# tenstack/batch-scheduler

Hardware: AMD Instinct MI355X
Metric: pod x node fit evals/sec (higher is better)
Workload: dtype int64; 1 GPU; cfg3/tail: 10000 pods / 2000 groups / 5000 nodes, 5 int64 lanes (cpu, mem, eph, pods, gpu), seed 20260921; stages=prefilter+filter+tally+ready, parallelism=single GPU

## Files before the change

### batch-scheduler_amd/csrc/bs_fast.hpp

```cpp
#pragma once

#include "bs_kernels.hpp"
#include "bs_filter_t.hpp"

#ifdef BS_NT_TABLES
#define BS_TBL_STORE(p, v) __builtin_nontemporal_store((v), (p))
#else
#define BS_TBL_STORE(p, v) (*(p) = (v))
#endif
namespace bs {

template <bool INL = false>
__device__ __forceinline__ void arm_tally(const GroupsDev& gr, const BatchDev& b, const BatchParams& prm, uint32_t i, uint32_t nthreads);

__device__ __forceinline__ const uint8_t* range_glocal(const BatchDev& b) { return reinterpret_cast<const uint8_t*>(b.pod_ranges); }
__device__ __forceinline__ const uint32_t* range_start(const BatchDev& b, uint32_t G) { return b.pod_ranges + (G + 3u) / 4u; }
__device__ __forceinline__ const uint32_t* range_lfirst(const BatchDev& b, uint32_t G, uint32_t pod_blocks) { return range_start(b, G) + pod_blocks + 1u; }
__device__ __forceinline__ bool range_local_on(const BatchDev& b, const BatchParams& prm) {
  return b.pod_ranges && prm.do_tally && prm.do_ready && !prm.filter_deny;
}

#if BS_EMIT_MAIN
__global__ void k_pods_prep(unsigned long long* tables, uint32_t ntab, uint32_t* gstat, uint32_t ngstat, uint32_t* kcount, uint32_t* gcount, uint32_t G) {
  const uint32_t t = blockIdx.x * blockDim.x + threadIdx.x, nt = gridDim.x * blockDim.x;
// ... 476 lines not shown
    if (have && lp.have_mr) res_add(ms, lp.mr, sh, gate);
    uint32_t ff = (have && lp.have_mr) ? 1u : 0u;
#pragma unroll
    for (uint32_t q = 0; q < BS_MAX_SCALARS; ++q)
      if (q < sh.S() && (ms.present & (1u << q)) && ms.v[4 + q] != 0) ff |= 2u;
    const unsigned long long holds = __ballot(l[0] >= ms.v[0] && l[1] >= ms.v[1] && l[2] >= ms.v[2] && l[3] >= ms.v[3]);
    if (stores) {
      b.nodew[nodew_pair(stride, s, w)] = ok;
      b.nodew[nodew_pair(stride, s, w) + 1] = ~holds;
    }
    if (blk == 0 && threadIdx.x == 0) {
#pragma unroll
      for (int j = 0; j < 4; ++j) b.nodew[nodew_ref_lane(stride, s, j)] = (uint64_t)ms.v[j];
      b.nodew[nodew_ref_flags(stride, s)] = ff;
    }
  }
}

template <int TS>
__global__ __launch_bounds__(kTblChunk) void k_fast_query_tables(PodsDev pods, GroupsDev gr, NodesDev nd, BatchDev b, BatchDev bt, BatchParams prm,
                                                                 const TableDesc* forced, uint32_t nchunks, uint32_t query_blocks) {
  BS_STAMP(1, 0);
  if (blockIdx.x < query_blocks) fast_query_thread<TS>(pods, gr, b, prm, blockIdx.x * kTblChunk + threadIdx.x, query_blocks * kTblChunk);
  else if (blockIdx.x < query_blocks + nchunks) tables_local_fast<TS>(nd, bt, prm, forced, blockIdx.x - query_blocks);
  else node_words_block<TS>(gr, nd, b, prm, blockIdx.x - query_blocks - nchunks);
  BS_STAMP(1, 7);
}

template <int NL>
__device__ __forceinline__ unsigned long long rows_cover(unsigned long long m, const int64_t (&a)[BS_MAX_LANES], const int64_t (&r)[BS_MAX_LANES]) {
  asm volatile("s_mov_b64 exec, %[m]\n\tv_cmpx_ge_i64 vcc, %[a0], %[r0]\n\tv_cmpx_ge_i64 vcc, %[a1], %[r1]\n\tv_cmpx_ge_i64 vcc, %[a2], %[r2]\n\t"
               "v_cmpx_ge_i64 vcc, %[a3], %[r3]\n\ts_mov_b64 %[m], exec\n\ts_mov_b64 exec, -1"
               : [m] "+s"(m)
               : [a0] "v"(a[0]), [r0] "v"(r[0]), [a1] "v"(a[1]), [r1] "v"(r[1]), [a2] "v"(a[2]), [r2] "v"(r[2]), [a3] "v"(a[3]), [r3] "v"(r[3])
               : "vcc");
#pragma unroll
  for (int j = 4; j < NL; ++j)
    asm volatile("s_mov_b64 exec, %[m]\n\tv_cmpx_ge_i64 vcc, %[a], %[r]\n\ts_mov_b64 %[m], exec\n\ts_mov_b64 exec, -1" : [m] "+s"(m) : [a] "v"(a[j]), [r] "v"(r[j]) : "vcc");
  return m;
}
#ifndef BS_SCAN_BALLOT
#define BS_SCAN_BALLOT 1
#endif
constexpr uint32_t kSpinBound = 1u << 18;
__device__ __forceinline__ void test_chaos_delay() {
#ifdef BS_TEST_CHAOS
  uint32_t h = (blockIdx.x + 1u) * 2654435761u ^ (uint32_t)wall_clock64() * 40503u;
  h ^= h >> 15; h *= 2246822519u; h ^= h >> 13;
  for (uint32_t s = 0; s < (h & 15u); ++s) __builtin_amdgcn_s_sleep(127);
#endif
}
constexpr uint32_t kStepSlotsMax = 256;
__device__ __forceinline__ bool step_wait(const uint32_t* word, uint32_t base, uint32_t need, int32_t* h_err) {
  uint32_t spins = 0;
  while ((uint32_t)(ld_agent(word) - base) < need) {
    __builtin_amdgcn_s_sleep(1);
    if (++spins > kSpinBound) { if (h_err) __hip_atomic_store(h_err, 1, __ATOMIC_RELAXED, __HIP_MEMORY_SCOPE_SYSTEM); return false; }
  }
  return true;
}
constexpr uint32_t kScanRecChunks = 64;
constexpr uint32_t kFeasRecGroups = 32;
#ifndef BS_GATHER_DIRECT
#define BS_GATHER_DIRECT 8
#endif
constexpr uint32_t kGatherDirectBlocks = BS_GATHER_DIRECT;
constexpr uint32_t kRecStride = 32;
constexpr uint32_t kTkSlots = 32, kTkTab = 48, kTkP1 = 64, kTkDone = 64 + 16 * 16, kTkWays = 16, kTkWords = 64 + 2 * 16 * 16;
__device__ __forceinline__ void spread_add(uint32_t* words, uint32_t who) {
  (void)__hip_atomic_fetch_add(&words[16u * (who % kTkWays)], 1u, __ATOMIC_RELAXED, __HIP_MEMORY_SCOPE_AGENT);
}
__device__ __forceinline__ bool spread_wait(const uint32_t* words, uint32_t base, uint32_t need, int32_t* h_err) {
  uint32_t spins = 0;
  for (;;) {
    uint32_t v = lane_id() < (int)kTkWays ? ld_agent(&words[16u * (uint32_t)lane_id()]) : 0u;
#pragma unroll
    for (int o = 1; o < (int)kTkWays; o <<= 1) v += (uint32_t)__shfl_xor((int)v, o);
    v = (uint32_t)__builtin_amdgcn_readfirstlane((int)v);
    if ((uint32_t)(v - base) >= need) return true;
    __builtin_amdgcn_s_sleep(4);
    if (++spins > kSpinBound) { if (h_err && lane_id() == 0) __hip_atomic_store(h_err, 1, __ATOMIC_RELAXED, __HIP_MEMORY_SCOPE_SYSTEM); return false; }
  }
}
template <int TS, bool REGS = false>
__device__ __forceinline__ void table_scan_block(const NodesDev& nd, const BatchDev& b, const BatchParams& prm, const TableDesc* forced, uint32_t chunk, uint32_t nchunks,
                                                 uint32_t share, uint32_t nshares, uint32_t pod_blocks, uint32_t tk_pods0, uint32_t tk_tab0, const GroupsDev& gr,
                                                 const int64_t* ckeys, const uint32_t* cpres, uint32_t kcap, bool direct = false, uint32_t forced_cls = 0) {
  __shared__ unsigned long long s_wtot[BS_MAX_LANES][4];
  __shared__ uint32_t s_kp[BS_MAX_SCALARS];
  __shared__ unsigned long long s_off[BS_MAX_LANES];
  __shared__ uint32_t s_kpg[BS_MAX_SCALARS];
  __shared__ int64_t s_req[kStepSlotsMax][BS_MAX_LANES];
  __shared__ uint32_t s_qf[kStepSlotsMax];
  __shared__ uint32_t s_first[kStepSlotsMax];
  BS_STAMP(2, 0);
  const Shape<TS> sh(prm.S);
  const uint32_t L = sh.L(), S = sh.S(), LP = prm.LP;
  const uint32_t k = chunk * kTblChunk + threadIdx.x;
  const bool in_range = REGS ? k < nd.n : k < nd.m;
  const uint32_t n = REGS ? (in_range ? k : 0u) : (in_range ? nd.kmap[k] : 0u);
  const TableDesc d = REGS ? TableDesc{forced_cls, 0.7f} : *forced;
  const uint32_t fw = nd.fit[(size_t)d.cls * nd.fit_words + (n >> 5)];
  const uint8_t fl = nd.flags[n];
  const bool valid = in_range && (!REGS || !(fl & BS_NODE_SKIP_MASK));
  const uint32_t ap = nd.apres[n], rp = nd.rpres[n];
  int64_t al[BS_MAX_LANES], rq[BS_MAX_LANES];
#pragma unroll
  for (uint32_t j = 0; j < BS_MAX_LANES; ++j) {
    if (j < L) {
      al[j] = nd.alloc[(size_t)j * nd.stride + n];
      rq[j] = nd.req[(size_t)j * nd.stride + n];
    }
  }
  const uint32_t K = prm.k_host ? prm.k_host : *b.kclass;
  const uint32_t per = (K + nshares - 1u) / nshares, s_lo = share * per, s_hi = min(K, s_lo + per);
  Res raw;
  int32_t leader0 = -1;
  uint8_t panic0 = 0;
  LeaderPre lp0{};
  if constexpr (REGS) {
    const uint32_t cc = s_lo + threadIdx.x < s_hi ? s_lo + threadIdx.x : 0u;
#pragma unroll
    for (uint32_t j = 0; j < BS_MAX_LANES; ++j)
      if (j < L) raw.v[j] = ckeys[(size_t)j * kcap + cc];
    raw.present = cpres[cc];
    leader0 = b.leader_epoch[0];
    panic0 = b.panic_epoch[0];
    if (gr.g) leader_pre_load(gr, leader0, sh, lp0);
  }
  const bool fit = valid && ((fw >> (n & 31u)) & 1u) && !(fl & BS_NODE_TAINT_ERR);
  const uint32_t pres = fit ? (ap & rp) : 0u;
  if (threadIdx.x < BS_MAX_SCALARS) s_kp[threadIdx.x] = BS_INF;
  for (uint32_t t = threadIdx.x; t < kStepSlotsMax; t += kTblChunk) s_first[t] = BS_INF;
  unsigned long long incl[BS_MAX_LANES];
  const int w = wave_id();
#pragma unroll
  for (uint32_t j = 0; j < BS_MAX_LANES; ++j) {
    incl[j] = 0;
    if (j < L) {
      const bool live = fit && (j < 4 || (pres & (1u << (j - 4)))) && !(j == BS_LANE_EPH && !prm.eph_gate);
      const unsigned long long left = live ? (unsigned long long)wsub(scale_f32(al[j], d.pct), rq[j]) : 0ull;
      incl[j] = wave_incl_scan_add_u64(left);
      if (lane_id() == 63) s_wtot[j][w] = incl[j];
    }
  }
  __syncthreads();
#pragma unroll
  for (uint32_t s2 = 0; s2 < BS_MAX_SCALARS; ++s2) {
    if (s2 < S) {
      const unsigned long long mk = __ballot(valid && (pres & (1u << s2)));
      if (mk && lane_id() == 0) atomicMin(&s_kp[s2], chunk * kTblChunk + (uint32_t)(threadIdx.x & ~63u) + (uint32_t)(__ffsll((long long)mk) - 1));
    }
  }
#pragma unroll
  for (uint32_t j = 0; j < BS_MAX_LANES; ++j) {
    if (j < L) {
      unsigned long long off = 0, tot = 0;
#pragma unroll
      for (int i = 0; i < 4; ++i) {
        const unsigned long long x = s_wtot[j][i];
        if (i < w) off += x;
        tot += x;
      }
      incl[j] += off;
      if (threadIdx.x == 0 && share == 0) {
        if constexpr (REGS) {
          const unsigned long long tag = (unsigned long long)prm.seq_inv << 32;
          st_pub<true>(&b.chunk_rec[(size_t)chunk * kRecStride + 2u * j], tag | (uint32_t)tot);
          st_pub<true>(&b.chunk_rec[(size_t)chunk * kRecStride + 2u * j + 1u], tag | (uint32_t)(tot >> 32));
        } else {
          st_pub<true>(&b.chunk_tot[(size_t)chunk * 16 + j], tot);
        }
      }
    }
  }
  __syncthreads();
  __shared__ uint32_t s_ok;
  if constexpr (REGS) {
    if (share == 0 && threadIdx.x < S) st_pub<true>(&b.chunk_rec[(size_t)chunk * kRecStride + 16u + threadIdx.x], ((unsigned long long)prm.seq_inv << 32) | s_kp[threadIdx.x]);
    BS_STAMP(2, 1);
  } else {
    if (share == 0 && threadIdx.x < 16) st_pub<true>(&b.chunk_kp[(size_t)chunk * 16 + threadIdx.x], threadIdx.x < BS_MAX_SCALARS ? s_kp[threadIdx.x] : BS_INF);
    asm volatile("s_waitcnt vmcnt(0)" ::: "memory");
    __syncthreads();
    BS_STAMP(2, 1);
    if (threadIdx.x == 0 && share == 0) (void)__hip_atomic_fetch_add(&b.ticket[kTkTab], 1u, __ATOMIC_RELAXED, __HIP_MEMORY_SCOPE_AGENT);
  }
  if constexpr (REGS) {
    const uint32_t t = s_lo + threadIdx.x;
    if (t < s_hi) {
      uint32_t qf = 0x80000000u;
      Res q;
      res_zero(q, sh);
      if (leader0 >= 0 && !panic0) {
        Res cur;
        res_zero(cur, sh);
        res_add(cur, raw, sh, prm.eph_gate);
        qf = class_scan_query(cur, lp0, sh, prm.eph_gate, q);
      }
      s_qf[threadIdx.x] = qf;
#pragma unroll
      for (uint32_t j = 0; j < BS_MAX_LANES; ++j)
        if (j < L) s_req[threadIdx.x][j] = q.v[j];
    }
  }
  if constexpr (!REGS) {
    if (threadIdx.x == 0) s_ok = (step_wait(&b.ticket[kTkTab], tk_tab0, nchunks, b.h_err) && step_wait(&b.ticket[kTkSlots], tk_pods0, pod_blocks, b.h_err)) ? 1u : 0u;
    __syncthreads();
    BS_STAMP(2, 2);
    if (!s_ok) return;
  }
  {
    const uint32_t ch = (uint32_t)lane_id();
    unsigned long long cv[BS_MAX_LANES];
    uint32_t ckp[BS_MAX_SCALARS];
    if constexpr (REGS) {
      if (w == 0) {
        const uint32_t tagw = prm.seq_inv;
        const unsigned long long* rec = b.chunk_rec + (size_t)(ch < nchunks ? ch : 0u) * kRecStride;
        bool ok = false;
        for (uint32_t spins = 0;; ++spins) {
          unsigned long long lo[BS_MAX_LANES], hi[BS_MAX_LANES], kw[BS_MAX_SCALARS];
#pragma unroll
          for (uint32_t j = 0; j < BS_MAX_LANES; ++j)
            if (j < L) { lo[j] = ld_agent64(&rec[2u * j]); hi[j] = ld_agent64(&rec[2u * j + 1u]); }
#pragma unroll
          for (uint32_t s2 = 0; s2 < BS_MAX_SCALARS; ++s2)
            if (s2 < S) kw[s2] = ld_agent64(&rec[16u + s2]);
          bool mine_ok = true;
#pragma unroll
          for (uint32_t j = 0; j < BS_MAX_LANES; ++j) {
            cv[j] = 0ull;
            if (j < L) {
              mine_ok = mine_ok && (uint32_t)(lo[j] >> 32) == tagw && (uint32_t)(hi[j] >> 32) == tagw;
              cv[j] = (hi[j] << 32) | (uint32_t)lo[j];
            }
          }
#pragma unroll
          for (uint32_t s2 = 0; s2 < BS_MAX_SCALARS; ++s2) {
            ckp[s2] = BS_INF;
            if (s2 < S) { mine_ok = mine_ok && (uint32_t)(kw[s2] >> 32) == tagw; ckp[s2] = (uint32_t)kw[s2]; }
          }
          if (__ballot(!(mine_ok || ch >= nchunks)) == 0ull) { ok = true; break; }
          if (spins > kSpinBound) { if (b.h_err && ch == 0) __hip_atomic_store(b.h_err, 1, __ATOMIC_RELAXED, __HIP_MEMORY_SCOPE_SYSTEM); break; }
          __builtin_amdgcn_s_sleep(2);
        }
        if (ch >= nchunks) {
#pragma unroll
          for (uint32_t j = 0; j < BS_MAX_LANES; ++j) cv[j] = 0ull;
#pragma unroll
          for (uint32_t s2 = 0; s2 < BS_MAX_SCALARS; ++s2) ckp[s2] = BS_INF;
        }
        if (ch == 0) s_ok = ok ? 1u : 0u;
      }
      BS_STAMP(2, 2);
    } else if (w == 0) {
#pragma unroll
      for (uint32_t j = 0; j < BS_MAX_LANES; ++j) cv[j] = (j < L && ch < nchunks) ? ld_agent64(&b.chunk_tot[(size_t)ch * 16 + j]) : 0ull;
#pragma unroll
      for (uint32_t s2 = 0; s2 < BS_MAX_SCALARS; ++s2) ckp[s2] = (s2 < S && ch < nchunks) ? ld_agent(&b.chunk_kp[(size_t)ch * 16 + s2]) : BS_INF;
    }
    const uint32_t t = s_lo + threadIdx.x;
    uint32_t stp = 0, qf = 0x80000000u;
    int32_t tab = -1;
    unsigned long long rv[BS_MAX_LANES];
    if (!REGS && t < s_hi) {
      stp = ld_agent(&b.qstamp_s[t]);
      tab = (int32_t)ld_agent(reinterpret_cast<const uint32_t*>(&b.qtab_s[t]));
      qf = ld_agent(&b.qflags_s[t]);
#pragma unroll
      for (uint32_t j = 0; j < BS_MAX_LANES; ++j) rv[j] = j < L ? ld_agent64(&b.qreq_s[(size_t)t * LP + j]) : 0ull;
    }
    if (w == 0) {
#pragma unroll
      for (uint32_t j = 0; j < BS_MAX_LANES; ++j) {
        if (j < L) {
          const unsigned long long incl_c = wave_incl_scan_add_u64(cv[j]);
          const unsigned long long mine = bcast64(incl_c - cv[j], (int)(chunk & 63u));
          if (ch == 0) s_off[j] = mine;
        }
      }
#pragma unroll
      for (uint32_t s2 = 0; s2 < BS_MAX_SCALARS; ++s2) {
        if (s2 < S) {
          const uint32_t mn = wave_min_u32(ckp[s2]);
          if (ch == 0) s_kpg[s2] = mn;
        }
      }
    }
    if (!REGS && t < s_hi) {
      if (stp != prm.stamp || tab != 0) qf = 0x80000000u;
      s_qf[threadIdx.x] = qf;
#pragma unroll
      for (uint32_t j = 0; j < BS_MAX_LANES; ++j)
        if (j < L) s_req[threadIdx.x][j] = (int64_t)rv[j];
    }
  }
  __syncthreads();
  if constexpr (REGS) {
    if (!s_ok) return;
  }
  int64_t fin[BS_MAX_LANES];
  uint32_t keyrow = 0;
#pragma unroll
  for (uint32_t j = 0; j < BS_MAX_LANES; ++j) {
    fin[j] = 0;
    if (j < L) fin[j] = (int64_t)(incl[j] + s_off[j]);
  }
#pragma unroll
  for (uint32_t s2 = 0; s2 < BS_MAX_SCALARS; ++s2)
    if (s2 < S && k >= s_kpg[s2]) keyrow |= 1u << s2;
  BS_STAMP(2, 3);
  const uint32_t nmine = s_hi > s_lo ? s_hi - s_lo : 0u;
  const uint32_t smask = S ? ((1u << S) - 1u) : 0u;
  const uint32_t row0 = chunk * kTblChunk + ((uint32_t)w << 6);
  for (uint32_t t0 = 0; t0 < nmine; t0 += 4u) {
    uint32_t qf[4];
    int64_t r[4][BS_MAX_LANES];
#pragma unroll
    for (uint32_t u = 0; u < 4; ++u) {
      const uint32_t t = min(t0 + u, nmine - 1u);
      qf[u] = t0 + u < nmine ? s_qf[t] : 0x80000000u;
#pragma unroll
      for (uint32_t j = 0; j < BS_MAX_LANES; ++j) r[u][j] = j < L ? s_req[t][j] : 0;
    }
#pragma unroll
    for (uint32_t u = 0; u < 4; ++u) {
      const uint32_t nab = ~(qf[u] >> 16) & smask;
      unsigned long long m = (qf[u] & 0x80000000u) ? 0ull : __ballot(valid && (nab & ~keyrow) == 0u);
      static_assert(TS >= 0 && TS <= 4, "k_fast_step_a is instantiated for 0..4 scalar lanes (run_fast: step_a_possible)");
#if BS_SCAN_BALLOT
#pragma unroll
      for (uint32_t j = 0; j < 4u + (uint32_t)TS; ++j) m &= __ballot(fin[j] >= r[u][j]);
#else
      m = rows_cover<4 + TS>(m, fin, r[u]);
#endif
      if (m && lane_id() == 0) atomicMin(&s_first[t0 + u], row0 + (uint32_t)(__ffsll((long long)m) - 1));
    }
  }
  __syncthreads();
  BS_STAMP(2, 4);
  if constexpr (REGS) {
    if (direct) {
      for (uint32_t t = threadIdx.x; t < nmine; t += kTblChunk)
        st_pub<true>(&b.scan_rec[(size_t)chunk * kStepSlotsMax + s_lo + t], ((unsigned long long)prm.seq_inv << 32) | s_first[t]);
    } else {
      for (uint32_t t = threadIdx.x; t < nmine; t += kTblChunk)
        if (s_first[t] != BS_INF) atomicMin(&b.first_row64[s_lo + t], ((unsigned long long)prm.seq_inv << 32) | s_first[t]);
    }
    BS_STAMP(2, 7);
    return;
  }
  for (uint32_t t = threadIdx.x; t < nmine; t += kTblChunk) {
    if (s_first[t] == BS_INF) continue;
    atomicMin(&b.first_row[s_lo + t], s_first[t]);
  }
  BS_STAMP(2, 7);
}

__device__ __forceinline__ void step_filter_split(uint32_t K, uint32_t W, uint32_t target_waves, uint32_t& tiles, uint32_t& bpw, uint32_t& nchunk) {
  tiles = (2u * K + 63u) / 64u;
  uint32_t nsplit = max(1u, target_waves / max(tiles, 1u));
  nsplit = min(nsplit, max((W + 1u) / 2u, 1u));
  bpw = max(2u, (((W + nsplit - 1u) / nsplit + 1u) / 2u) * 2u);
  nchunk = (W + bpw - 1u) / bpw;
  if ((nchunk + 3u) / 4u > kFeasRecGroups) {
    bpw = ((W + 4u * kFeasRecGroups - 1u) / (4u * kFeasRecGroups) + 1u) / 2u * 2u;
    nchunk = (W + bpw - 1u) / bpw;
  }
}
template <int TS>
__device__ __forceinline__ void step_filter_block(const GroupsDev& gr, const NodesDev& nd, const BatchDev& b, const BatchParams& prm, const int64_t* ckeys,
                                                  const uint32_t* cpres, uint32_t kcap, uint32_t target_waves, uint32_t ustride, uint32_t bx, uint32_t nblocks,
                                                  bool direct, uint32_t tk_slots0, uint32_t slot_producers) {
  __shared__ uint32_t s_cnt[4][64];
  BS_STAMP_AT(4, 0, bx);
  const Shape<TS> sh(prm.S);
  const uint32_t gate = prm.eph_gate, K = prm.k_host ? prm.k_host : (uint32_t)__builtin_amdgcn_readfirstlane((int)*b.kclass), U = 2u * K;
  const uint32_t W = (nd.n + 63u) / 64u;
  if (!U || !W) return;
  uint32_t tiles, bpw, nchunk;
  step_filter_split(K, W, target_waves, tiles, bpw, nchunk);
  const uint32_t groups = (nchunk + 3u) / 4u;
  const int32_t leader0 = b.leader_epoch[0];
  LeaderPre lp0{}, lp1{};
  const bool two = prm.sop_leader0 >= 0 && prm.sop_leader0 != leader0;
  if (gr.g) {
    leader_pre_load(gr, leader0, sh, lp0);
    if (two) leader_pre_load(gr, prm.sop_leader0, sh, lp1); else lp1 = lp0;
  }
  bool waited = false;
  for (uint32_t bi = bx; bi < tiles * groups; bi += nblocks) {
    const uint32_t tile = bi % tiles, group = bi / tiles, chunk = group * 4u + (uint32_t)wave_id();
    const uint32_t src = tile * 64u + (uint32_t)lane_id();
    const bool second = src >= K;
    const uint32_t c = src < U ? (second ? src - K : src) : 0u;
    uint32_t cnt = 0;
    if (chunk < nchunk) {
      Res raw;
#pragma unroll
      for (uint32_t j = 0; j < BS_MAX_LANES; ++j)
        if (j < sh.L()) raw.v[j] = ckeys[(size_t)j * kcap + c];
      raw.present = cpres[c];
      Res cur;
      res_zero(cur, sh);
      res_add(cur, raw, sh, gate);
      LeaderPre lp = lp0;
      if (second) lp = lp1;
      const bool on = src < U && (second ? prm.sop_leader0 >= 0 : leader0 >= 0) && lp.have_mr;
      int64_t R[4], M[4];
      const uint32_t ff = filter_slot_values(cur, lp, sh, gate, R, M);
      filter_item<2, 4, true, true>(nd, b, U, ustride, tile, chunk * bpw, min(W, chunk * bpw + bpw), 0u,
                                    on ? (ff | ((uint32_t)BS_FL_EVALUATED << 8)) : ((uint32_t)BS_FL_NOT_RUN << 8), R, M, &cnt);
    }
    s_cnt[wave_id()][lane_id()] = cnt;
    BS_STAMP_AT(4, 1, bx);
    if (direct && b.h_rows) asm volatile("s_waitcnt vmcnt(0)" ::: "memory");
    __syncthreads();
    BS_STAMP_AT(4, 2, bx);
    if (wave_id() == 0 && src < U) {
      const uint32_t sum = s_cnt[0][lane_id()] + s_cnt[1][lane_id()] + s_cnt[2][lane_id()] + s_cnt[3][lane_id()];
      if (direct) {
        st_pub<true>(&b.feas_rec[(size_t)group * (2u * kStepSlotsMax) + src], ((unsigned long long)prm.seq_inv << 32) | sum);
      } else {
        if (!waited) { (void)step_wait(&b.ticket[kTkSlots], tk_slots0, slot_producers, b.h_err); waited = true; }
        if (sum) atomicAdd(&b.fu_feas[src], sum);
      }
    }
    __syncthreads();
  }
  BS_STAMP_AT(4, 7, bx);
}

template <int TS>
__device__ __forceinline__ void class_slots_block(const GroupsDev& gr, const BatchDev& b, const BatchParams& prm, const int64_t* ckeys, const uint32_t* cpres,
                                                  uint32_t kcap, uint32_t blk, bool zero_feas) {
  const Shape<TS> sh(prm.S);
#ifdef BS_TEST_OLD_ZERO
  zero_feas = true;
#endif
  const uint32_t gate = prm.eph_gate, K = prm.k_host ? prm.k_host : *b.kclass;
  const uint32_t c = blk * kTblChunk + threadIdx.x;
  Res raw;
  const uint32_t cc = c < K ? c : 0u;
#pragma unroll
  for (uint32_t j = 0; j < BS_MAX_LANES; ++j)
    if (j < sh.L()) raw.v[j] = ckeys[(size_t)j * kcap + cc];
  raw.present = cpres[cc];
  const int32_t leader0 = b.leader_epoch[0];
  const uint8_t panic0 = b.panic_epoch[0];
  LeaderPre lp0{}, lp1{};
  const bool two = prm.run_filter && prm.sop_leader0 >= 0 && prm.sop_leader0 != leader0;
  if (gr.g) {
    leader_pre_load(gr, leader0, sh, lp0);
    if (two) leader_pre_load(gr, prm.sop_leader0, sh, lp1); else lp1 = lp0;
  }
  if (c < K) {
    Res cur;
    res_zero(cur, sh);
    res_add(cur, raw, sh, gate);
    if (leader0 >= 0 && !panic0) {
      Res q;
      const uint32_t qfw = class_scan_query(cur, lp0, sh, gate, q);
      int64_t* dst = b.qreq_s + (size_t)c * prm.LP;
#pragma unroll
      for (uint32_t j = 0; j < BS_MAX_LANES; ++j)
        if (j < prm.LP) st_pub<true>(&dst[j], j < sh.L() ? q.v[j] : (int64_t)INT64_MIN);
      st_pub<true>(&b.qflags_s[c], qfw);
      st_pub<true>(&b.qtab_s[c], (int32_t)0);
      st_pub<true>(&b.first_row[c], BS_INF);
      st_pub<true>(&b.qstamp_s[c], prm.stamp);
    }
    if (prm.run_filter) {
      if (leader0 >= 0) filter_slot_from<TS, true>(b, prm, cur, lp0, sh, gate, c, zero_feas);
      if (prm.sop_leader0 >= 0) filter_slot_from<TS, true>(b, prm, cur, lp1, sh, gate, c + K, zero_feas);
    }
  }
  BS_STAMP(1, 4);
  asm volatile("s_waitcnt vmcnt(0)" ::: "memory");
  __syncthreads();
  BS_STAMP(1, 5);
  if (threadIdx.x == 0) (void)__hip_atomic_fetch_add(&b.ticket[kTkSlots], 1u, __ATOMIC_RELAXED, __HIP_MEMORY_SCOPE_AGENT);
}


template <bool INL>
__device__ __forceinline__ void arm_tally(const GroupsDev& gr, const BatchDev& b, const BatchParams& prm, uint32_t i, uint32_t nthreads) {
  if (i == 0) __hip_atomic_store(&b.ticket[1], 0u, __ATOMIC_RELAXED, __HIP_MEMORY_SCOPE_AGENT);
  for (uint32_t g = i; g < gr.g; g += nthreads) {
    if (INL && range_local_on(b, prm) && range_glocal(b)[g]) continue;
    st_pub<INL>(&b.admit[g], 0u);
    if (prm.do_ready) {
      st_pub<INL>(&b.admit64[g], 0ull);
      if (b.gcount[g] == 0u) {
        const uint8_t rd = gr.matched[g] >= (uint32_t)(gr.min_member[g] - gr.status_scheduled[g]) ? 1 : 0;
        b.ready[g] = rd;
        if (prm.host_tag) { st_home(&b.h_admit[g], 0u); st_home(&b.h_ready[g], rd); }
      }
    }
  }
}

template <bool WT = false>
__device__ __forceinline__ void final_tail(const BatchDev& b, const BatchParams& prm, uint32_t nblocks) {
  __shared__ uint32_t s_last;
  if (!prm.host_tag) return;
  if constexpr (WT && BS_HOME_WT) asm volatile("s_waitcnt vmcnt(0)" ::: "memory");
  else __builtin_amdgcn_fence(__ATOMIC_RELEASE, "");
// ... 292 lines not shown
      tally_tail<true>(gr, b, prm, grouped, grouped ? (uint32_t)gi0 : 0u, admit, nblocks);
  }
  BS_STAMP(3, 7);
}

template <int S>
__global__ __launch_bounds__(256) void k_fast_scan_filter(PodsDev pods, NodesDev nd, BatchDev bt, BatchParams prm, uint32_t m, uint32_t jcap,
                                                          uint32_t scan_blocks, uint32_t filter_waves, uint32_t ustride) {
  __shared__ int64_t s_rows[4][64][4 + S];
  if (blockIdx.x < scan_blocks)
    scan_loop<S, true, 1>(bt, prm, m, jcap, 0u, 0u, 1u, blockIdx.x, scan_blocks, s_rows[wave_id()]);
  else
    filter_loop<2>(pods, nd, bt, filter_waves, 1u, ustride, prm.collect_stats, blockIdx.x - scan_blocks, gridDim.x - scan_blocks, prm.stamp, 2u * prm.k_host);
}
template <int S>
__global__ __launch_bounds__(256) void k_fast_scan(BatchDev bt, BatchParams prm, uint32_t m, uint32_t jcap) {
  __shared__ int64_t s_rows[4][64][4 + S];
  scan_loop<S, true, 1>(bt, prm, m, jcap, 0u, 0u, 1u, blockIdx.x, gridDim.x, s_rows[wave_id()]);
}
template <int PU, bool DB>
__global__ __launch_bounds__(256) void k_fast_filter(PodsDev pods, NodesDev nd, BatchDev bt, BatchParams prm, uint32_t filter_waves, uint32_t ustride) {
  filter_loop<2, PU, DB>(pods, nd, bt, filter_waves, 1u, ustride, prm.collect_stats, blockIdx.x, gridDim.x, prm.stamp, 2u * prm.k_host);
}
#if BS_EMIT_FAST
__global__ __launch_bounds__(256) __attribute__((amdgpu_waves_per_eu(7))) void k_fast_filter_w7(PodsDev pods, NodesDev nd, BatchDev bt, BatchParams prm, uint32_t filter_waves,
                                                                                                uint32_t ustride) {
  filter_loop<2, 2, false>(pods, nd, bt, filter_waves, 1u, ustride, prm.collect_stats, blockIdx.x, gridDim.x, prm.stamp, 2u * prm.k_host);
}
#endif
#if BS_EMIT_FAST
__global__ __launch_bounds__(256) void k_fast_filter_t(NodesDev nd, BatchDev bt, BatchParams prm, uint32_t filter_waves, uint32_t ustride, uint32_t by_tile) {
  filter_loop_t<false>(nd, bt, filter_waves, ustride, prm.collect_stats, blockIdx.x, gridDim.x, prm.stamp, 2u * prm.k_host, by_tile);
}
#endif
template <int S>
__global__ __launch_bounds__(256) __attribute__((amdgpu_waves_per_eu(S <= 1 ? 4 : 1))) void k_fast_scan_filter_t(NodesDev nd, BatchDev bt, BatchParams prm, uint32_t m, uint32_t jcap, uint32_t scan_blocks,
                                                            uint32_t filter_waves, uint32_t ustride, uint32_t form) {
  __shared__ int64_t s_rows[4][64][4 + S];
  const uint32_t filter_first = form & 1u, by_tile = form & 2u;
  const uint32_t filter_blocks = gridDim.x - scan_blocks;
  const bool is_scan = filter_first ? blockIdx.x >= filter_blocks : blockIdx.x < scan_blocks;
  BS_STAMP(2, 0);
  if (is_scan)
    scan_loop<S, true, 1>(bt, prm, m, jcap, 0u, 0u, 1u, filter_first ? blockIdx.x - filter_blocks : blockIdx.x, scan_blocks, s_rows[wave_id()]);
  else
    filter_loop_t<true>(nd, bt, filter_waves, ustride, prm.collect_stats, filter_first ? blockIdx.x : blockIdx.x - scan_blocks, filter_blocks, prm.stamp, 2u * prm.k_host, by_tile);
  BS_STAMP(2, 7);
}
#if BS_EMIT_MAIN
__global__ __launch_bounds__(256) void k_fast_final(PodsDev pods, GroupsDev gr, NodesDev nd, BatchDev b, BatchParams prm, uint32_t query_blocks) {
  fast_final_block(pods, gr, nd, b, prm, query_blocks, blockIdx.x, gridDim.x, 0u);
}
#endif

template <int S>
__global__ __launch_bounds__(256) void k_fast_scan_filter_final(PodsDev pods, GroupsDev gr, NodesDev nd, BatchDev b, BatchDev bt, BatchParams prm, uint32_t m,
                                                                uint32_t jcap, uint32_t scan_blocks, uint32_t filter_blocks, uint32_t filter_waves,
                                                                uint32_t ustride, uint32_t query_blocks) {
  __shared__ int64_t s_rows[4][64][4 + S];
  const uint32_t producers = scan_blocks + filter_blocks;
  test_chaos_delay();
#ifdef BS_TEST_LATE_ROLE_B
  {
    const int role = blockIdx.x < scan_blocks ? 0 : blockIdx.x < producers ? 1 : 2;
    if (role == BS_TEST_LATE_ROLE_B) for (int spin = 0; spin < 20; ++spin) __builtin_amdgcn_s_sleep(127);
  }
#endif
  if (blockIdx.x < producers) {
    BS_STAMP(2, 0);
    if (blockIdx.x < scan_blocks)
      scan_loop<S, true, 2>(bt, prm, m, jcap, 0u, 0u, 1u, blockIdx.x, scan_blocks, s_rows[wave_id()]);
    else
      filter_loop<2>(pods, nd, bt, filter_waves, 1u, ustride, prm.collect_stats, blockIdx.x - scan_blocks, filter_blocks, prm.stamp, 2u * prm.k_host);
    asm volatile("s_waitcnt vmcnt(0)" ::: "memory");
    __syncthreads();
    if (threadIdx.x == 0) (void)__hip_atomic_fetch_add(&b.ticket[1], 1u, __ATOMIC_RELAXED, __HIP_MEMORY_SCOPE_AGENT);
    BS_STAMP(2, 7);
    return;
  }
  fast_final_block(pods, gr, nd, b, prm, query_blocks, blockIdx.x - producers, gridDim.x - producers, producers);
}

template <int TS, bool WHOLE>
__global__ __launch_bounds__(kTblChunk) void k_fast_step_a(PodsDev pods, GroupsDev gr, NodesDev nd, BatchDev b, BatchDev bt, BatchParams prm, const TableDesc* forced,
                                                           uint32_t nchunks, uint32_t query_blocks, uint32_t nshares, uint32_t filter_blocks, uint32_t filter_waves,
                                                           uint32_t ustride, uint32_t tk_pods0, uint32_t tk_tab0, uint32_t param_blocks, const int64_t* ckeys,
                                                           const uint32_t* cpres, uint32_t kcap, uint32_t tk_p1, uint32_t tk_done, uint32_t forced_cls) {
  BS_STAMP(1, 0);
  test_chaos_delay();
  const uint32_t tb = nchunks * nshares;
#ifdef BS_TEST_LATE_ROLE
  {
    const int role = blockIdx.x < query_blocks ? 0 : blockIdx.x < query_blocks + param_blocks ? 1 : blockIdx.x < query_blocks + param_blocks + tb ? 2 : 3;
    if (role == BS_TEST_LATE_ROLE) for (int spin = 0; spin < 20; ++spin) __builtin_amdgcn_s_sleep(127);
  }
#endif
  const uint32_t producers = param_blocks ? param_blocks : query_blocks;
  const bool direct = query_blocks <= kGatherDirectBlocks;
  if (blockIdx.x < query_blocks) {
    if constexpr (WHOLE) {
      const uint32_t p0 = b.pod_ranges ? range_start(b, gr.g)[blockIdx.x] : blockIdx.x * kTblChunk;
      const uint32_t p1 = b.pod_ranges ? range_start(b, gr.g)[blockIdx.x + 1u] : pods.p;
      fast_query_thread<TS, false, false, true>(pods, gr, b, prm, p0 + threadIdx.x, query_blocks * kTblChunk, p1, blockIdx.x * kTblChunk + threadIdx.x);
      asm volatile("s_waitcnt vmcnt(0)" ::: "memory");
      __syncthreads();
      if (threadIdx.x == 0) spread_add(&b.ticket[kTkP1], blockIdx.x);
      fast_final_block<true>(pods, gr, nd, b, prm, query_blocks, blockIdx.x, query_blocks, nchunks, tk_p1, filter_waves, tk_done, tb + filter_blocks, p0, p1);
    } else if (param_blocks) {
      fast_query_thread<TS, false, false>(pods, gr, b, prm, blockIdx.x * kTblChunk + threadIdx.x, query_blocks * kTblChunk);
    } else {
      fast_query_thread<TS, true>(pods, gr, b, prm, blockIdx.x * kTblChunk + threadIdx.x, query_blocks * kTblChunk);
      BS_STAMP(1, 4);
      asm volatile("s_waitcnt vmcnt(0)" ::: "memory");
      __syncthreads();
      BS_STAMP(1, 5);
      if (threadIdx.x == 0) (void)__hip_atomic_fetch_add(&b.ticket[kTkSlots], 1u, __ATOMIC_RELAXED, __HIP_MEMORY_SCOPE_AGENT);
    }
  } else if (blockIdx.x < query_blocks + param_blocks) {
    class_slots_block<TS>(gr, b, prm, ckeys, cpres, kcap, blockIdx.x - query_blocks, !(WHOLE && direct));
  } else if (blockIdx.x < query_blocks + param_blocks + tb) {
    const uint32_t x = blockIdx.x - query_blocks - param_blocks;
    table_scan_block<TS, WHOLE>(nd, bt, prm, forced, x / nshares, nchunks, x % nshares, nshares, producers, tk_pods0, tk_tab0, gr, ckeys, cpres, kcap, direct, forced_cls);
    if constexpr (WHOLE) {
      if (!direct) {
        asm volatile("s_waitcnt vmcnt(0)" ::: "memory");
        __syncthreads();
        if (threadIdx.x == 0) spread_add(&b.ticket[kTkDone], blockIdx.x);
      }
    }
  } else if constexpr (WHOLE) {
    step_filter_block<TS>(gr, nd, bt, prm, ckeys, cpres, kcap, filter_waves, ustride, blockIdx.x - query_blocks - param_blocks - tb, filter_blocks, direct, tk_pods0, producers);
    if (!direct) {
      asm volatile("s_waitcnt vmcnt(0)" ::: "memory");
      __syncthreads();
      if (threadIdx.x == 0) spread_add(&b.ticket[kTkDone], blockIdx.x);
    }
  } else {
    __shared__ uint32_t s_go;
    if (threadIdx.x == 0) {
      s_go = step_wait(&b.ticket[kTkSlots], tk_pods0, producers, b.h_err) ? 1u : 0u;
      __builtin_amdgcn_fence(__ATOMIC_ACQUIRE, "agent");
    }
    __syncthreads();
    if (!s_go) return;
    filter_loop<2>(pods, nd, bt, filter_waves, 1u, ustride, prm.collect_stats, blockIdx.x - query_blocks - param_blocks - tb, filter_blocks, prm.stamp, 2u * prm.k_host);
  }
  BS_STAMP(1, 7);
}


template <int TS>
__global__ __launch_bounds__(kTblChunk) void k_tables_local_nofix(NodesDev nd, BatchDev b, BatchParams prm, uint32_t nchunks, uint32_t cstride,
                                                                  uint32_t gstride) {
  const uint32_t slot = blockIdx.x;
  if (!b.needed[slot]) return;
  BatchDev bt = b;
  bt.tables = b.tables + (size_t)slot * prm.mcap * prm.LP;
  bt.kp = b.kp + (size_t)slot * 16;
  bt.chunk_tot = b.chunk_tot + (size_t)slot * cstride * 16;
  bt.chunk_kp = b.chunk_kp + (size_t)slot * cstride * 16;
  bt.gmax = b.gmax + (size_t)slot * gstride * prm.LP;
  const TableDesc d = table_desc(slot, prm.C, nullptr);
  tables_local_fast<TS>(nd, bt, prm, &d, blockIdx.y);
}

#if BS_EMIT_MAIN
__global__ __launch_bounds__(kLeaderBlock) void k_leader_scan(GroupsDev gr, BatchDev b) {
// ... 93 lines not shown
```

### batch-scheduler_amd/csrc/bs_kernels.hpp

```cpp
#pragma once

#include "bs_common.hpp"
#include "bs_nodew_layout.hpp"

namespace bs {

struct NodesDev {
  uint32_t n, stride;
  const int64_t* alloc;
  const int64_t* req;
  const uint32_t* apres;
  const uint32_t* rpres;
  const uint8_t* flags;
  const uint32_t* fit;
  uint32_t fit_words, n_classes;
  const uint32_t* kmap;
  uint32_t m;
  const int64_t* left4;
  const int64_t* lglob;
};

struct GroupsDev {
  uint32_t g;
  const uint32_t* min_member;
// ... 1486 lines not shown
__global__ void k_filter_params(PodsDev pods, GroupsDev gr, BatchDev b, BatchParams prm) {
  const uint32_t i = blockIdx.x * blockDim.x + threadIdx.x;
  if (i >= pods.p) return;
  filter_params_for<-1>(pods, gr, b, prm, i, b.pf_code[i], b.pf_leader[i], i, true, true);
}
#endif

template <int TS>
__global__ void k_fparams_early(PodsDev pods, GroupsDev gr, BatchDev b, BatchParams prm) {
  const uint32_t i = blockIdx.x * blockDim.x + threadIdx.x;
  if (i >= pods.p) return;
  const uint8_t pf = (b.stage[i] & ST_OWNED) ? b.tcode[i] : (uint8_t)BS_PF_NOT_OWNED;
  const bool after = i >= b.nepochs[1];
  const int32_t leader = after ? b.leader_epoch[0] : prm.sop_leader0;
  const uint32_t slot = prm.use_classes ? b.pclass[i] + (after ? 0u : *b.kclass) : i;
  filter_params_for<TS>(pods, gr, b, prm, i, pf, leader, slot, true, true);
}

#define BS_OPT_0(x) ""
#define BS_OPT_1(x) x
#define BS_OPT(flag, x) BS_OPT_##flag(x)
template <int MASK>
__device__ __forceinline__ void filter_pod2(uint32_t pp, const int64_t (&R)[4], unsigned long long ok0, unsigned long long ok1,
                                            const int64_t (&l0)[4], const int64_t (&l1)[4], uint32_t& vlo0, uint32_t& vhi0,
                                            uint32_t& vlo1, uint32_t& vhi1);
#define BS_DEF_FILTER_POD2(MASK, f0, f1, f2, f3)                                                                          \
  template <>                                                                                                             \
  __device__ __forceinline__ void filter_pod2<MASK>(uint32_t pp, const int64_t (&R)[4], unsigned long long ok0,          \
                                                    unsigned long long ok1, const int64_t (&l0)[4], const int64_t (&l1)[4], \
                                                    uint32_t& vlo0, uint32_t& vhi0, uint32_t& vlo1, uint32_t& vhi1) {       \
    asm volatile("s_mov_b32 m0, %[pp]\n\t"                                                                                \
                 "s_mov_b64 exec, %[ok0]\n\t"                                                                             \
                 BS_OPT(f0, "v_cmpx_le_i64 vcc, %[R0], %[a0]\n\t") BS_OPT(f1, "v_cmpx_le_i64 vcc, %[R1], %[a1]\n\t")       \
                 BS_OPT(f2, "v_cmpx_le_i64 vcc, %[R2], %[a2]\n\t") BS_OPT(f3, "v_cmpx_le_i64 vcc, %[R3], %[a3]\n\t")       \
                 "s_nop 3\n\t"                                                                                            \
                 "v_writelane_b32 %[vlo0], exec_lo, m0\n\t"                                                               \
                 "v_writelane_b32 %[vhi0], exec_hi, m0\n\t"                                                               \
                 "s_mov_b64 exec, %[ok1]\n\t"                                                                             \
                 BS_OPT(f0, "v_cmpx_le_i64 vcc, %[R0], %[b0]\n\t") BS_OPT(f1, "v_cmpx_le_i64 vcc, %[R1], %[b1]\n\t")       \
                 BS_OPT(f2, "v_cmpx_le_i64 vcc, %[R2], %[b2]\n\t") BS_OPT(f3, "v_cmpx_le_i64 vcc, %[R3], %[b3]\n\t")       \
                 "s_nop 3\n\t"                                                                                            \
                 "v_writelane_b32 %[vlo1], exec_lo, m0\n\t"                                                               \
                 "v_writelane_b32 %[vhi1], exec_hi, m0\n\t"                                                               \
                 "s_mov_b64 exec, -1"                                                                                     \
                 : [vlo0] "+v"(vlo0), [vhi0] "+v"(vhi0), [vlo1] "+v"(vlo1), [vhi1] "+v"(vhi1)                             \
                 : [pp] "s"(pp), [ok0] "s"(ok0), [ok1] "s"(ok1), [R0] "v"(R[0]), [R1] "v"(R[1]), [R2] "v"(R[2]),          \
                   [R3] "v"(R[3]), [a0] "v"(l0[0]), [a1] "v"(l0[1]), [a2] "v"(l0[2]), [a3] "v"(l0[3]), [b0] "v"(l1[0]),   \
                   [b1] "v"(l1[1]), [b2] "v"(l1[2]), [b3] "v"(l1[3])                                                      \
                 : "vcc");                                                                                                \
  }
BS_DEF_FILTER_POD2(1, 1, 0, 0, 0)
BS_DEF_FILTER_POD2(2, 0, 1, 0, 0)
BS_DEF_FILTER_POD2(3, 1, 1, 0, 0)
BS_DEF_FILTER_POD2(4, 0, 0, 1, 0)
BS_DEF_FILTER_POD2(5, 1, 0, 1, 0)
BS_DEF_FILTER_POD2(6, 0, 1, 1, 0)
BS_DEF_FILTER_POD2(7, 1, 1, 1, 0)
BS_DEF_FILTER_POD2(8, 0, 0, 0, 1)
BS_DEF_FILTER_POD2(9, 1, 0, 0, 1)
BS_DEF_FILTER_POD2(10, 0, 1, 0, 1)
BS_DEF_FILTER_POD2(11, 1, 1, 0, 1)
BS_DEF_FILTER_POD2(12, 0, 0, 1, 1)
BS_DEF_FILTER_POD2(13, 1, 0, 1, 1)
BS_DEF_FILTER_POD2(14, 0, 1, 1, 1)
BS_DEF_FILTER_POD2(15, 1, 1, 1, 1)

template <int MASK, int PU = 4>
__device__ __forceinline__ void filter_pod_loop(uint32_t np, const int64_t (*sR)[4], const unsigned long long (&okmask)[2],
                                                const int64_t (&l)[2][4], uint32_t (&vlo)[2], uint32_t (&vhi)[2]) {
  for (uint32_t pp = 0; pp < np; pp += PU) {
    int64_t R[PU][4];
#pragma unroll
    for (int u = 0; u < PU; ++u) {
      const uint32_t pu = min(pp + (uint32_t)u, np - 1);
#pragma unroll
      for (int j = 0; j < 4; ++j) R[u][j] = ((MASK >> j) & 1) ? sR[pu][j] : 0;
    }
#pragma unroll
    for (int u = 0; u < PU; ++u)
      filter_pod2<MASK>(min(pp + (uint32_t)u, np - 1), R[u], okmask[0], okmask[1], l[0], l[1], vlo[0], vhi[0], vlo[1], vhi[1]);
  }
}

template <int NB, int PU = 4, bool DB = true, bool REGS = false>
__device__ __forceinline__ void filter_item(const NodesDev& nd, const BatchDev& b, uint32_t U, uint32_t ustride, uint32_t ptile,
                                            uint32_t w0, uint32_t w1, uint32_t stamp = 0, uint32_t ff_in = 0, const int64_t* R_in = nullptr,
                                            const int64_t* M_in = nullptr, uint32_t* cnt_out = nullptr) {
  static_assert(NB == 2, "the inner statement handles two node blocks");
  typedef const __attribute__((address_space(4))) uint32_t* cflag_t;
  const int lane = lane_id();
  const uint32_t p0 = ptile * 64u;
  const uint32_t np = min(64u, U - p0);

  const bool mine = (uint32_t)lane < np;
  const uint32_t src = p0 + (uint32_t)lane;
  uint32_t myff = (uint32_t)BS_FL_NOT_RUN << 8;
  int64_t M[4] = {0, 0, 0, 0}, myR[4] = {0, 0, 0, 0};
  if constexpr (REGS) {
    if (mine) {
      myff = ff_in;
#pragma unroll
      for (int j = 0; j < 4; ++j) { myR[j] = R_in[j]; M[j] = M_in[j]; }
    }
  } else if (mine) {
    myff = b.uflags[src];
    const int64_t* rs = b.uparams + (size_t)src * 8;
#pragma unroll
    for (int j = 0; j < 4; ++j) { myR[j] = rs[j]; M[j] = rs[4 + j]; }
  }
  int64_t gl[8];
#pragma unroll
  for (int j = 0; j < 8; ++j) gl[j] = nd.lglob[j];
  int64_t l[NB][4], ln[NB][4];
  uint8_t nfl[NB], nfln[NB];
  auto load_blocks = [&](uint32_t w, int64_t (&dst)[NB][4], uint8_t (&fl)[NB]) {
#pragma unroll
    for (int nb = 0; nb < NB; ++nb) {
      const uint32_t n = (w + nb) * 64u + (uint32_t)lane;
      const bool nvalid = (w + nb) < w1 && n < nd.n;
      fl[nb] = 0xFF;
#pragma unroll
      for (int j = 0; j < 4; ++j) dst[nb][j] = INT64_MIN;
      if (nvalid) {
#pragma unroll
        for (int j = 0; j < 4; ++j) dst[nb][j] = nd.left4[(size_t)j * nd.stride + n];
        fl[nb] = nd.flags[n];
      }
    }
  };
  load_blocks(w0, l, nfl);
  if (!REGS && stamp) myff = (myff >> 16) == stamp ? (myff & 0xFFFFu) : ((uint32_t)BS_FL_NOT_RUN << 8);
  const uint32_t myfl = myff >> 8;
  const bool ev = myfl == BS_FL_EVALUATED;
  if (!ev) {
#pragma unroll
    for (int j = 0; j < 4; ++j) M[j] = 0;
  }
  __shared__ int64_t s_R[4][64][4];
  __builtin_amdgcn_wave_barrier();
  uint32_t lane_mask = 0;
  bool tile_allfail = false;
  {
#pragma unroll
    for (int j = 0; j < 4; ++j) s_R[wave_id()][lane][j] = myR[j];
    __builtin_amdgcn_wave_barrier();
    const bool c2pod = ev && !(myff & 1u);
    const unsigned long long c2mask = __ballot(c2pod);
#pragma unroll
    for (int j = 0; j < 4; ++j) {
      if (__ballot(c2pod && !(gl[j] >= myR[j]))) lane_mask |= 1u << j;
      if (c2mask && !__ballot(c2pod && gl[4 + j] >= myR[j])) tile_allfail = true;
    }
  }
  const unsigned long long evmask = __ballot(ev);
  if (!evmask) return;
  bool uniformM = true;
  int64_t M0[4] = {0, 0, 0, 0};
  uint32_t lb0 = 0;
  if (evmask) {
    const int first = __ffsll((long long)evmask) - 1;
    bool same = true;
#pragma unroll
    for (int j = 0; j < 4; ++j) {
      M0[j] = __shfl(M[j], first);
      same = same && (M[j] == M0[j]);
    }
    lb0 = (uint32_t)__shfl((int)(myff & 2u), first);
    same = same && ((myff & 2u) == lb0);
    uniformM = __ballot(ev && !same) == 0;
  }

  crow_t FP = as_const_rows(b.uparams);
  cflag_t FF = (cflag_t)(uintptr_t)b.uflags;
  uint32_t cnt = 0;
  for (uint32_t w = w0; w < w1; w += NB) {
    if constexpr (DB) {
      if (w + NB < w1) load_blocks(w + NB, ln, nfln);
    }
    unsigned long long okmask[NB], in_range[NB], nlf[NB];
    uint32_t vlo[NB], vhi[NB];
#pragma unroll
    for (int nb = 0; nb < NB; ++nb) {
      const bool nvalid = nfl[nb] != 0xFF;
      const bool node_ok = nvalid && !(nfl[nb] & (BS_NODE_NIL | BS_NODE_NO_NODE));
      in_range[nb] = __ballot(nvalid);
      okmask[nb] = __ballot(node_ok);
      unsigned long long lf = 0;
      if (!lb0) lf = __ballot(l[nb][0] >= M0[0]) & __ballot(l[nb][1] >= M0[1]) & __ballot(l[nb][2] >= M0[2]) & __ballot(l[nb][3] >= M0[3]);
      nlf[nb] = okmask[nb] & ~lf;
      vlo[nb] = 0;
      vhi[nb] = 0;
    }
    if (uniformM) {
      const int64_t (*sR)[4] = s_R[wave_id()];
      if (tile_allfail) {
      } else {
        switch (lane_mask) {
          case 0:
#pragma unroll
            for (int nb = 0; nb < NB; ++nb) { vlo[nb] = (uint32_t)okmask[nb]; vhi[nb] = (uint32_t)(okmask[nb] >> 32); }
            break;
          case 1: filter_pod_loop<1, PU>(np, sR, okmask, l, vlo, vhi); break;
          case 2: filter_pod_loop<2, PU>(np, sR, okmask, l, vlo, vhi); break;
          case 3: filter_pod_loop<3, PU>(np, sR, okmask, l, vlo, vhi); break;
          case 4: filter_pod_loop<4, PU>(np, sR, okmask, l, vlo, vhi); break;
          case 5: filter_pod_loop<5, PU>(np, sR, okmask, l, vlo, vhi); break;
          case 6: filter_pod_loop<6, PU>(np, sR, okmask, l, vlo, vhi); break;
          case 7: filter_pod_loop<7, PU>(np, sR, okmask, l, vlo, vhi); break;
          case 8: filter_pod_loop<8, PU>(np, sR, okmask, l, vlo, vhi); break;
          case 9: filter_pod_loop<9, PU>(np, sR, okmask, l, vlo, vhi); break;
          case 10: filter_pod_loop<10, PU>(np, sR, okmask, l, vlo, vhi); break;
          case 11: filter_pod_loop<11, PU>(np, sR, okmask, l, vlo, vhi); break;
          case 12: filter_pod_loop<12, PU>(np, sR, okmask, l, vlo, vhi); break;
// ... 281 lines not shown
```

Measured before the change: 3765 billion evals/s.

## Restructure step-A table scan with lane-distributed requests and prefetch filter inputs

In the REGS table-scan path, each lane now holds one pod request in registers, and the wave broadcasts it with readlane instead of rereading shared memory for every pod. Per-pod first-row results are collected into a lane via v_writelane and committed with one atomicMin per lane, replacing one atomic per pod. The filter loop also prefetches pod keys and node blocks for the next item before the leader preload and before waiting on the ticket, and it skips the spin-wait when an early ticket read already shows all producers are done. The kernel is additionally hinted to run at 3 waves per EU, which could cause register spills or lower occupancy.

```diff
diff --git a/batch-scheduler_amd/csrc/bs_fast.hpp b/batch-scheduler_amd/csrc/bs_fast.hpp
--- a/batch-scheduler_amd/csrc/bs_fast.hpp
+++ b/batch-scheduler_amd/csrc/bs_fast.hpp
@@ -582,6 +582,13 @@
     if (++spins > kSpinBound) { if (h_err && lane_id() == 0) __hip_atomic_store(h_err, 1, __ATOMIC_RELAXED, __HIP_MEMORY_SCOPE_SYSTEM); return false; }
   }
 }
+#pragma clang diagnostic push
+#pragma clang diagnostic ignored "-Winline-asm"
+__device__ __forceinline__ uint32_t writelane_sgpr(uint32_t value, int lane, uint32_t old) {
+  asm("s_mov_b32 m0, %2\n\tv_writelane_b32 %0, %1, m0" : "+v"(old) : "s"(value), "s"(lane) : "m0");
+  return old;
+}
+#pragma clang diagnostic pop
 template <int TS, bool REGS = false>
 __device__ __forceinline__ void table_scan_block(const NodesDev& nd, const BatchDev& b, const BatchParams& prm, const TableDesc* forced, uint32_t chunk, uint32_t nchunks,
                                                  uint32_t share, uint32_t nshares, uint32_t pod_blocks, uint32_t tk_pods0, uint32_t tk_tab0, const GroupsDev& gr,
@@ -704,6 +711,24 @@
         if (j < L) s_req[threadIdx.x][j] = q.v[j];
     }
   }
+  const uint32_t nmine = (uint32_t)__builtin_amdgcn_readfirstlane((int)(s_hi > s_lo ? s_hi - s_lo : 0u));
+  const uint32_t smask = S ? ((1u << S) - 1u) : 0u;
+  static_assert(TS >= 0 && TS <= 4, "k_fast_step_a is instantiated for 0..4 scalar lanes (run_fast: step_a_possible)");
+  constexpr uint32_t NL = 4u + (uint32_t)TS;
+  int64_t rr[NL];
+  uint32_t nabx = 0;
+  [[maybe_unused]] auto req_round = [&](uint32_t base) {
+    const uint32_t t = base + (uint32_t)lane_id();
+    const bool have = t < nmine;
+    const uint32_t qf = have ? s_qf[t] : 0x80000000u;
+#pragma unroll
+    for (uint32_t j = 0; j < NL; ++j) rr[j] = have ? s_req[t][j] : 0;
+    nabx = (qf & 0x80000000u) ? 0xC0000000u : ((~(qf >> 16) & smask) | 0x80000000u);
+  };
+  if constexpr (REGS) {
+    __syncthreads();
+    req_round(0u);
+  }
   if constexpr (!REGS) {
     if (threadIdx.x == 0) s_ok = (step_wait(&b.ticket[kTkTab], tk_tab0, nchunks, b.h_err) && step_wait(&b.ticket[kTkSlots], tk_pods0, pod_blocks, b.h_err)) ? 1u : 0u;
     __syncthreads();
@@ -811,9 +836,32 @@
   for (uint32_t s2 = 0; s2 < BS_MAX_SCALARS; ++s2)
     if (s2 < S && k >= s_kpg[s2]) keyrow |= 1u << s2;
   BS_STAMP(2, 3);
-  const uint32_t nmine = s_hi > s_lo ? s_hi - s_lo : 0u;
-  const uint32_t smask = S ? ((1u << S) - 1u) : 0u;
-  const uint32_t row0 = chunk * kTblChunk + ((uint32_t)w << 6);
+  const uint32_t row0 = (uint32_t)__builtin_amdgcn_readfirstlane((int)(chunk * kTblChunk + ((uint32_t)w << 6)));
+  if constexpr (REGS) {
+    constexpr uint32_t kU = TS <= 1 ? 8u : 4u;
+    const uint32_t rowbits = valid ? ((~keyrow & smask) | 0x40000000u) : ~0u;
+    for (uint32_t base = 0; base < nmine; base += 64u) {
+      if (base) req_round(base);
+      const uint32_t cnt = min(64u, nmine - base);
+      uint32_t first = BS_INF;
+      for (uint32_t s0 = 0; s0 < cnt; s0 += kU) {
+#pragma unroll
+        for (uint32_t u = 0; u < kU; ++u) {
+          const int sl = (int)(s0 + u);
+          unsigned long long m = __ballot(((uint32_t)__builtin_amdgcn_readlane((int)nabx, sl) & rowbits) == 0u);
+#pragma unroll
+          for (uint32_t j = 0; j < NL; ++j) {
+            const int64_t r = (int64_t)(((unsigned long long)(uint32_t)__builtin_amdgcn_readlane((int)((unsigned long long)rr[j] >> 32), sl) << 32) |
+                                        (uint32_t)__builtin_amdgcn_readlane((int)(uint32_t)rr[j], sl));
+            m &= __ballot(fin[j] >= r);
+          }
+          const uint32_t row = m ? row0 + (uint32_t)(__ffsll((long long)m) - 1) : BS_INF;
+          first = writelane_sgpr(row, sl, first);
+        }
+      }
+      if ((uint32_t)lane_id() < cnt && first != BS_INF) atomicMin(&s_first[base + (uint32_t)lane_id()], first);
+    }
+  } else {
   for (uint32_t t0 = 0; t0 < nmine; t0 += 4u) {
     uint32_t qf[4];
     int64_t r[4][BS_MAX_LANES];
@@ -837,6 +885,7 @@
 #endif
       if (m && lane_id() == 0) atomicMin(&s_first[t0 + u], row0 + (uint32_t)(__ffsll((long long)m) - 1));
     }
+  }
   }
   __syncthreads();
   BS_STAMP(2, 4);
@@ -883,25 +932,36 @@
   step_filter_split(K, W, target_waves, tiles, bpw, nchunk);
   const uint32_t groups = (nchunk + 3u) / 4u;
   const int32_t leader0 = b.leader_epoch[0];
+  Res raw;
+  FilterPre<2> pre;
+  auto item_load = [&](uint32_t bi) {
+    const uint32_t tile = bi % tiles, chunk = (bi / tiles) * 4u + (uint32_t)wave_id();
+    const uint32_t src = tile * 64u + (uint32_t)lane_id();
+    const uint32_t c = src < U ? (src >= K ? src - K : src) : 0u;
+#pragma unroll
+    for (uint32_t j = 0; j < BS_MAX_LANES; ++j)
+      if (j < sh.L()) raw.v[j] = ckeys[(size_t)j * kcap + c];
+    raw.present = cpres[c];
+    filter_node_blocks<2>(nd, chunk * bpw, chunk < nchunk ? min(W, chunk * bpw + bpw) : 0u, pre.l, pre.nfl);
+  };
+#pragma unroll
+  for (int j = 0; j < 8; ++j) pre.gl[j] = nd.lglob[j];
+  item_load(min(bx, tiles * groups - 1u));
+  const uint32_t tk_early = direct ? 0u : ld_agent(&b.ticket[kTkSlots]);
+  bool waited = false;
   LeaderPre lp0{}, lp1{};
   const bool two = prm.sop_leader0 >= 0 && prm.sop_leader0 != leader0;
   if (gr.g) {
     leader_pre_load(gr, leader0, sh, lp0);
     if (two) leader_pre_load(gr, prm.sop_leader0, sh, lp1); else lp1 = lp0;
   }
-  bool waited = false;
   for (uint32_t bi = bx; bi < tiles * groups; bi += nblocks) {
     const uint32_t tile = bi % tiles, group = bi / tiles, chunk = group * 4u + (uint32_t)wave_id();
     const uint32_t src = tile * 64u + (uint32_t)lane_id();
     const bool second = src >= K;
-    const uint32_t c = src < U ? (second ? src - K : src) : 0u;
     uint32_t cnt = 0;
+    if (bi != bx) item_load(bi);
     if (chunk < nchunk) {
-      Res raw;
-#pragma unroll
-      for (uint32_t j = 0; j < BS_MAX_LANES; ++j)
-        if (j < sh.L()) raw.v[j] = ckeys[(size_t)j * kcap + c];
-      raw.present = cpres[c];
       Res cur;
       res_zero(cur, sh);
       res_add(cur, raw, sh, gate);
@@ -911,7 +971,7 @@
       int64_t R[4], M[4];
       const uint32_t ff = filter_slot_values(cur, lp, sh, gate, R, M);
       filter_item<2, 4, true, true>(nd, b, U, ustride, tile, chunk * bpw, min(W, chunk * bpw + bpw), 0u,
-                                    on ? (ff | ((uint32_t)BS_FL_EVALUATED << 8)) : ((uint32_t)BS_FL_NOT_RUN << 8), R, M, &cnt);
+                                    on ? (ff | ((uint32_t)BS_FL_EVALUATED << 8)) : ((uint32_t)BS_FL_NOT_RUN << 8), R, M, &cnt, &pre);
     }
     s_cnt[wave_id()][lane_id()] = cnt;
     BS_STAMP_AT(4, 1, bx);
@@ -923,7 +983,10 @@
       if (direct) {
         st_pub<true>(&b.feas_rec[(size_t)group * (2u * kStepSlotsMax) + src], ((unsigned long long)prm.seq_inv << 32) | sum);
       } else {
-        if (!waited) { (void)step_wait(&b.ticket[kTkSlots], tk_slots0, slot_producers, b.h_err); waited = true; }
+        if (!waited) {
+          if ((uint32_t)(tk_early - tk_slots0) < slot_producers) (void)step_wait(&b.ticket[kTkSlots], tk_slots0, slot_producers, b.h_err);
+          waited = true;
+        }
         if (sum) atomicAdd(&b.fu_feas[src], sum);
       }
     }
@@ -1382,7 +1445,7 @@
 }
 
 template <int TS, bool WHOLE>
-__global__ __launch_bounds__(kTblChunk) void k_fast_step_a(PodsDev pods, GroupsDev gr, NodesDev nd, BatchDev b, BatchDev bt, BatchParams prm, const TableDesc* forced,
+__global__ __launch_bounds__(kTblChunk) __attribute__((amdgpu_waves_per_eu(3))) void k_fast_step_a(PodsDev pods, GroupsDev gr, NodesDev nd, BatchDev b, BatchDev bt, BatchParams prm, const TableDesc* forced,
                                                            uint32_t nchunks, uint32_t query_blocks, uint32_t nshares, uint32_t filter_blocks, uint32_t filter_waves,
                                                            uint32_t ustride, uint32_t tk_pods0, uint32_t tk_tab0, uint32_t param_blocks, const int64_t* ckeys,
                                                            const uint32_t* cpres, uint32_t kcap, uint32_t tk_p1, uint32_t tk_done, uint32_t forced_cls) {
diff --git a/batch-scheduler_amd/csrc/bs_kernels.hpp b/batch-scheduler_amd/csrc/bs_kernels.hpp
--- a/batch-scheduler_amd/csrc/bs_kernels.hpp
+++ b/batch-scheduler_amd/csrc/bs_kernels.hpp
@@ -1592,10 +1592,32 @@
   }
 }
 
+template <int NB>
+struct FilterPre {
+  int64_t gl[8];
+  int64_t l[NB][4];
+  uint8_t nfl[NB];
+};
+template <int NB>
+__device__ __forceinline__ void filter_node_blocks(const NodesDev& nd, uint32_t w, uint32_t w1, int64_t (&dst)[NB][4], uint8_t (&fl)[NB]) {
+#pragma unroll
+  for (int nb = 0; nb < NB; ++nb) {
+    const uint32_t n = (w + nb) * 64u + (uint32_t)lane_id();
+    const bool nvalid = (w + nb) < w1 && n < nd.n;
+    fl[nb] = 0xFF;
+#pragma unroll
+    for (int j = 0; j < 4; ++j) dst[nb][j] = INT64_MIN;
+    if (nvalid) {
+#pragma unroll
+      for (int j = 0; j < 4; ++j) dst[nb][j] = nd.left4[(size_t)j * nd.stride + n];
+      fl[nb] = nd.flags[n];
+    }
+  }
+}
 template <int NB, int PU = 4, bool DB = true, bool REGS = false>
 __device__ __forceinline__ void filter_item(const NodesDev& nd, const BatchDev& b, uint32_t U, uint32_t ustride, uint32_t ptile,
                                             uint32_t w0, uint32_t w1, uint32_t stamp = 0, uint32_t ff_in = 0, const int64_t* R_in = nullptr,
-                                            const int64_t* M_in = nullptr, uint32_t* cnt_out = nullptr) {
+                                            const int64_t* M_in = nullptr, uint32_t* cnt_out = nullptr, const FilterPre<NB>* pre = nullptr) {
   static_assert(NB == 2, "the inner statement handles two node blocks");
   typedef const __attribute__((address_space(4))) uint32_t* cflag_t;
   const int lane = lane_id();
@@ -1620,7 +1642,10 @@
   }
   int64_t gl[8];
 #pragma unroll
-  for (int j = 0; j < 8; ++j) gl[j] = nd.lglob[j];
+  for (int j = 0; j < 8; ++j) {
+    if constexpr (REGS) gl[j] = pre->gl[j];
+    else gl[j] = nd.lglob[j];
+  }
   int64_t l[NB][4], ln[NB][4];
   uint8_t nfl[NB], nfln[NB];
   auto load_blocks = [&](uint32_t w, int64_t (&dst)[NB][4], uint8_t (&fl)[NB]) {
@@ -1638,7 +1663,16 @@
       }
     }
   };
-  load_blocks(w0, l, nfl);
+  if constexpr (REGS) {
+#pragma unroll
+    for (int nb = 0; nb < NB; ++nb) {
+      nfl[nb] = pre->nfl[nb];
+#pragma unroll
+      for (int j = 0; j < 4; ++j) l[nb][j] = pre->l[nb][j];
+    }
+  } else {
+    load_blocks(w0, l, nfl);
+  }
   if (!REGS && stamp) myff = (myff >> 16) == stamp ? (myff & 0xFFFFu) : ((uint32_t)BS_FL_NOT_RUN << 8);
   const uint32_t myfl = myff >> 8;
   const bool ev = myfl == BS_FL_EVALUATED;
```

Result: slower. 3634 billion evals/s (-3.5%).
